# tzjtatata/Myriad

Hardware: AMD Instinct MI355X
Metric: images/sec fine-tune step (Vicuna-7B + LoRA-style adapters, 224px) (higher is better)
Workload: dtype bf16

## Files before the change

### include/myriad_hip.h

```cpp
#ifndef MYRIAD_HIP_H
#define MYRIAD_HIP_H
#include <stdint.h>

#ifdef __cplusplus
extern "C" {
#endif

typedef struct ihipStream_t* mh_stream_t;

#define MH_OK 0
#define MH_ERR_ARG (-1)
#define MH_ERR_LAUNCH (-2)
#define MH_ERR_UNSUPPORTED (-3)

#define MH_GEMM_OUT_F32 1
#define MH_GEMM_GELU 2
#define MH_GEMM_REGSTAGE 4

int mh_gemm_bf16_nt(const void* A, int lda, const void* B, int ldb, void* C, int ldc, int M, int N, int K,
                    const float* bias, const float* residual, int ldr, int flags, float alpha, mh_stream_t s);

int mh_gemm_plan(int M, int N, int K, int flags, int* kernel, int* splits);

int mh_prof_start(int capacity, mh_stream_t s);
// ... 111 lines not shown
int mh_lora_refresh_border(const float* Bq, const float* Bv, void* ext, long ld_ext, void* extT, long ld_extT, int W,
                           int D, int r, mh_stream_t st);
int mh_lora_refresh_borders(const void* table, int n_layers, long ld_ext, long ld_extT, int W, int D, int r, mh_stream_t stream);

int mh_lowrank_fwd(const float* x, const float* A, const float* Bm, float* y, float* t, int M, int D, int R,
                   mh_stream_t s);
long mh_lowrank_bwd_ws_floats(int M, int D, int R);
int mh_lowrank_bwd(const float* dy, const float* x, const float* t, const float* A, const float* Bm, float* dA,
                   float* dB, float* dx, float* ws, int M, int D, int R, mh_stream_t s);

int mh_clamp_ce(const float* logits, long ldl, const long* labels, float* row_loss, void* dlogits_bf16, long ldd,
                int R, int V, float grad_scale, mh_stream_t s);
int mh_sum_f32(const float* x, float* out, long n, float scale, mh_stream_t s);
int mh_argmax_rows(const float* logits, long ldl, long* out, float* margin, int R, int V, int ban_id, mh_stream_t s);
int mh_argmax_pmax_rows(const float* logits, long ldl, long* out, float* margin, float* pmax, int R, int V, int ban_id,
                        float inv_temp, mh_stream_t s);
int mh_decode_record(const long* nxt, const float* margin, const float* pmax, float* rec, long* next_ids, int* step, int R,
                     mh_stream_t s);
int mh_decode_advance(const long* nxt, const float* margin, const float* pmax, float* rec, long* next_ids, int* step, int* pos,
                      int* kvlen, int R, mh_stream_t s);
int mh_sample_rows(const float* logits, long ldl, long* out, float* margin, float* pmax, int* kept, float* u_out, int R, int V,
                   int ban_id, const float* params, const unsigned long long* seed, const int* step, int t_add, mh_stream_t s);
int mh_repetition_penalty_rows(float* logits, long ldl, unsigned* seen, const long* prev_ids, int R, int V, const float* penalty,
                               mh_stream_t s);
int mh_decode_advance_kept(const long* nxt, const float* margin, const float* pmax, const int* kept, float* rec, long* next_ids,
                           int* step, int* pos, int* kvlen, int R, mh_stream_t s);
int mh_decode_advance_rows(const long* nxt, const float* margin, const float* pmax, float* rec, long* next_ids, int* step,
                           int* pos, int* kvlen, const int* live, int R, mh_stream_t s);
int mh_sample_rows_slots(const float* logits, long ldl, long* out, float* margin, float* pmax, int* kept, float* u_out, int R, int V,
                         const float* params, const unsigned long long* seed, const int* gen, const int* live, mh_stream_t s);
int mh_argmax_pmax_rows_slots(const float* logits, long ldl, long* out, float* margin, float* pmax, int R, int V, const float* params,
                              const int* gen, const int* live, mh_stream_t s);
int mh_repetition_penalty_rows_slots(float* logits, long ldl, unsigned* seen, const long* prev_ids, int R, int V, const float* penalty,
                                     const int* live, mh_stream_t s);
int mh_decode_advance_kept_rows(const long* nxt, const float* margin, const float* pmax, const int* kept, float* rec, long* next_ids,
                                int* step, int* pos, int* kvlen, int* gen, const int* live, int R, mh_stream_t s);
int mh_token_scores_rows(const float* logits, long ldl, const long* ids, const int* watch, float* out, long ldo, int R, int V,
                         const int* live, mh_stream_t s);

int mh_beam_topk(const float* logits, long ldl, const float* scores, float* part_s, int* part_i, float* out_s, int* out_i, int B,
                 int rpi, int nb, int V, int ban_id, int* pos, int* kvlen, int n_adv, mh_stream_t s);
int mh_beam_reorder_kv(void* const* caches, int L, int B, int nb, long T_cap, int C, const int* src, const int* lo, const int* hi,
                       mh_stream_t s);

int mh_im2col_nhwc(const void* x, void* col, int B, int H, int W, int C, int kh, int kw, int pad, int Kpad,
                   mh_stream_t s);
int mh_col2im_nhwc(const void* dcol, float* dx, int B, int H, int W, int C, int kh, int kw, int pad, int Kpad,
                   mh_stream_t s);
int mh_relu_maxpool2_fwd(const void* y, int y_is_f32, long ldy, void* p, int B, int H, int W, int C, mh_stream_t s);
int mh_relu_maxpool2_bwd(const float* dp, const void* y, int y_is_f32, long ldy, void* dy, long lddy, int B, int H,
                         int W, int C, mh_stream_t s);
int mh_conv_pack_weight(const float* W, const float* bias, void* Wp, int Cout, int K, int Kpad, mh_stream_t s);
int mh_conv_unpack_grad(const float* dWp, float* dW, float* db, int Cout, int K, int Kpad, mh_stream_t s);

int mh_embed_gather(const void* table_bf16, const long* ids, const int* dst_rows, float* out, long n, int D, long ldo,
                    mh_stream_t s);
int mh_copy2d_f32(const float* src, long lds, float* dst, long ldd, long rows, int cols, int accumulate,
                  mh_stream_t s);
int mh_copy3d_f32(const float* src, long src_bstride, long lds, float* dst, long dst_bstride, long ldd, int nb,
                  long rows, int cols, int accumulate, mh_stream_t s);
int mh_gather_rows_f32_to_bf16(const float* src, long lds, const int* rows, void* dst, long n, int D, mh_stream_t s);
int mh_gather_rows_f32(const float* src, long lds, const int* rows, float* dst, long n, int D, mh_stream_t s);
int mh_gather_rows(const void* src, long lds, const int* rows, void* dst, long n, int D, int elem_bytes, mh_stream_t s);
int mh_expand_rows(const void* src, const int* inv, void* dst, long ldd, long M, int D, int elem_bytes, mh_stream_t s);
int mh_copy3d_bf16(const void* src, long src_bstride, long lds, void* dst, long dst_bstride, long ldd, int nb,
                   long rows, int cols, mh_stream_t s);
int mh_kv_append_bf16(const void* src, long ld_src, void* cache, long cache_bstride, long ld_cache, const int* pos_dev,
                      int B, int cols, mh_stream_t s);
int mh_rope_kv_append(void* qkv, long ld, int n_heads, int head_dim, const int* pos, const float* cos_tab,
                      const float* sin_tab, void* cache, long cache_bstride, long ld_cache, const int* pos_dev, int B,
                      mh_stream_t s);
int mh_add_i32(int* x, int n, int delta, mh_stream_t s);
long mh_gemv_pack_elems(int N, int K);
int mh_gemv_pack(const void* W, int ldb, int N, int K, void* out, mh_stream_t s);
int mh_gemv_packed(const void* A, int lda, const void* P, void* C, int ldc, int M, int N, int K, const float* bias,
                   const float* residual, int ldr, int out_f32, float alpha, mh_stream_t s);
int mh_gemv_packed_rmsnorm(const float* H, long ldh, const float* norm_w, float eps, const void* P, void* C, int ldc, int M,
                           int N, int K, const float* bias, const float* residual, int ldr, int out_f32, float alpha,
                           mh_stream_t s);
int mh_gemv_packed_silu(const void* gu, long ldgu, const void* P, void* C, int ldc, int M, int N, int K, const float* bias,
                        const float* residual, int ldr, int out_f32, float alpha, mh_stream_t s);
long mh_gemv_pack_fp8_elems(int N, int K);
int mh_gemv_pack_fp8(const void* W, int ldb, int N, int K, void* q_out, float* scale_out, mh_stream_t s);
int mh_gemv_packed_fp8(const void* A, int lda, const void* Q, const float* scale, void* C, int ldc, int M, int N, int K,
                       const float* bias, const float* residual, int ldr, int out_f32, float alpha, mh_stream_t s);
int mh_gemv_packed_fp8_rmsnorm(const float* H, long ldh, const float* norm_w, float eps, const void* Q, const float* scale,
                               void* C, int ldc, int M, int N, int K, const float* bias, const float* residual, int ldr,
                               int out_f32, float alpha, mh_stream_t s);
int mh_gemv_packed_fp8_silu(const void* gu, long ldgu, const void* Q, const float* scale, void* C, int ldc, int M, int N, int K,
                            const float* bias, const float* residual, int ldr, int out_f32, float alpha, mh_stream_t s);
long mh_gemv_pack_fp4_elems(int N, int K);
long mh_gemv_pack_fp4_scale_elems(int N, int K);
int mh_gemv_pack_fp4(const void* W, int ldb, int N, int K, void* q_out, void* scale_out, mh_stream_t s);
int mh_gemv_packed_fp4(const void* A, int lda, const void* Q, const void* scale, void* C, int ldc, int M, int N, int K,
                       const float* bias, const float* residual, int ldr, int out_f32, float alpha, mh_stream_t s);
int mh_gemv_packed_fp4_rmsnorm(const float* H, long ldh, const float* norm_w, float eps, const void* Q, const void* scale,
                               void* C, int ldc, int M, int N, int K, const float* bias, const float* residual, int ldr,
                               int out_f32, float alpha, mh_stream_t s);
int mh_gemv_packed_fp4_silu(const void* gu, long ldgu, const void* Q, const void* scale, void* C, int ldc, int M, int N, int K,
                            const float* bias, const float* residual, int ldr, int out_f32, float alpha, mh_stream_t s);
int mh_gemv_packed_wide(const void* A, int lda, const void* P, void* C, int ldc, int M, int N, int K, const float* bias,
                        const float* residual, int ldr, int out_f32, float alpha, mh_stream_t s);
int mh_gemv_packed_fp8_wide(const void* A, int lda, const void* Q, const float* scale, void* C, int ldc, int M, int N, int K,
                            const float* bias, const float* residual, int ldr, int out_f32, float alpha, mh_stream_t s);
int mh_gemv_packed_fp4_wide(const void* A, int lda, const void* Q, const void* scale, void* C, int ldc, int M, int N, int K,
                            const float* bias, const float* residual, int ldr, int out_f32, float alpha, mh_stream_t s);
// ... 112 lines not shown
```

### myriad_amd/build.py

```python
from __future__ import annotations

import os
import subprocess
import sys
from concurrent.futures import ThreadPoolExecutor

HERE = os.path.dirname(os.path.abspath(__file__))
CSRC = os.path.join(HERE, "csrc")
OBJ = os.path.join(CSRC, "build")
LIB = os.path.join(HERE, "libmyriad_hip.so")
LIB_DBG = os.path.join(HERE, "libmyriad_hip_dbg.so")
DBG_SOURCES = ["gemm", "gemm_256", "gemm_x4", "attn_seq", "lora"]
SOURCES = ["gemm", "gemm_256", "gemm_x4", "gemv", "attention", "attn_decode_split", "attn_ragged", "attn_seq", "attn_full", "norm", "elementwise", "conv", "loss", "sample", "scores", "beam", "lowrank", "lora", "expert", "image", "selfsup", "optim", "prof", "ctx", "wgrad", "qf_dropout", "lora_merge", "refresh", "version"]
FLAGS = ["--offload-arch=gfx950", "-O3", "-std=c++17", "-fPIC", "-ffp-contract=fast"]


def _stale(out, deps):
    if not os.path.exists(out):
        return True
    t = os.path.getmtime(out)
    return any(os.path.getmtime(d) > t for d in deps)


def build(force: bool = False, verbose: bool = True) -> str:
    hipcc = os.environ.get("HIPCC", "/opt/rocm/bin/hipcc")
    os.makedirs(OBJ, exist_ok=True)
    hdrs = [os.path.join(CSRC, h) for h in ("common.h", "gemv_pack.h", "attn_frag.h", "attn_tile.h")]
    gen, inc = os.path.join(CSRC, "gen_gemm_x4.py"), os.path.join(CSRC, "gemm_x4_loop.inc")
    if force or _stale(inc, [gen]):
        subprocess.check_call([sys.executable, gen])
    hdrs.append(inc)

    def one(job):
        name, dbg = job
        src = os.path.join(CSRC, name + ".hip")
        obj = os.path.join(OBJ, name + (".dbg.o" if dbg else ".o"))
        if force or _stale(obj, [src, *hdrs]):
            cmd = [hipcc, *FLAGS, *(["-DMH_DEBUG_HOOKS"] if dbg else []), "-c", src, "-o", obj]
            if verbose:
                print(" ".join(cmd), flush=True)
            subprocess.check_call(cmd)
        return obj

    jobs = [(n, False) for n in SOURCES] + [(n, True) for n in DBG_SOURCES]
    with ThreadPoolExecutor(max_workers=min(8, len(jobs))) as ex:
        built = dict(zip(jobs, ex.map(one, jobs)))
    objs = [built[(n, False)] for n in SOURCES]
    objs_dbg = [built[(n, n in DBG_SOURCES)] for n in SOURCES]
    for lib, oo in ((LIB, objs), (LIB_DBG, objs_dbg)):
        if force or _stale(lib, oo):
            cmd = [hipcc, "--offload-arch=gfx950", "-shared", "-fPIC", "-o", lib, *oo, "-ldl"]
            if verbose:
                print(" ".join(cmd), flush=True)
            subprocess.check_call(cmd)
    return LIB


if __name__ == "__main__":
    print(build(force="--force" in sys.argv))
```

### myriad_amd/csrc/common.h

```cpp
#pragma once
#include <hip/hip_runtime.h>
#include <stdint.h>

#define MH_OK 0
#define MH_ERR_ARG (-1)
#define MH_ERR_LAUNCH (-2)
#define MH_ERR_UNSUPPORTED (-3)

typedef unsigned short bf16_t;
typedef __attribute__((ext_vector_type(8))) short short8_t;
typedef __attribute__((ext_vector_type(4))) short short4_t;
typedef __attribute__((ext_vector_type(4))) float float4_t;
typedef __attribute__((ext_vector_type(16))) float float16_t;

#define MH_CHECK_LAUNCH()                                   \
  do {                                                      \
    hipError_t e__ = hipGetLastError();                     \
    if (e__ != hipSuccess) return MH_ERR_LAUNCH;            \
  } while (0)

#define MH_MAX_ALT_WS 4
struct MhScratch {
  float* ws;
  size_t bytes;
  float* alt[MH_MAX_ALT_WS];
  hipStream_t alt_stream[MH_MAX_ALT_WS];
};
extern MhScratch g_default_scratch;
extern MhScratch* g_scratch;

enum MhOpt {
  MH_OPT_SLAB_BF16 = 0,
  MH_OPT_GEMM_SKINNY,
  MH_OPT_SWIGLU_FUSED,
  MH_OPT_GELU_FUSED,
  MH_OPT_ATTN_BWD_SPLIT,
  MH_OPT_GEMM_ZERO_PAD,
  MH_OPT_GEMM256_IMPL,
  MH_OPT_LORA_NORM_FUSED,
  MH_OPT_ATTN_FULL,
  MH_OPT_LORA_WGRAD_MFMA,
  MH_OPT_GEMM_SKIP_PAD,
  MH_OPT_GEMM_SPLIT_XCD,
  MH_OPT_COUNT
};
int mh_opt(int id);

extern bool g_mh_prof_on;
void mh_prof_pre(hipStream_t s, int kernel, int M, int N, int K, int splits, int flags);
void mh_prof_post(hipStream_t s);

__device__ __forceinline__ float bf2f(bf16_t h) { return __uint_as_float(((unsigned)h) << 16); }

typedef __bf16 mh_bf2_t __attribute__((ext_vector_type(2)));
typedef float mh_f2_t __attribute__((ext_vector_type(2)));
__device__ __forceinline__ bf16_t f2bf_sw(float f) {
  unsigned u = __float_as_uint(f);
  if ((u & 0x7fffffffu) > 0x7f800000u) return (bf16_t)((u >> 16) | 0x40);
  u += 0x7fffu + ((u >> 16) & 1u);
  return (bf16_t)(u >> 16);
}
__device__ __forceinline__ bf16_t f2bf(float f) {
  const __bf16 b = (__bf16)f;
  return (bf16_t)__builtin_bit_cast(unsigned short, b);
}
__device__ __forceinline__ unsigned pack_bf2(float lo, float hi) {
  const mh_f2_t v = {lo, hi};
  const mh_bf2_t b = __builtin_convertvector(v, mh_bf2_t);
  return __builtin_bit_cast(unsigned, b);
}

__device__ __forceinline__ unsigned dropout_hash(unsigned long long seed, unsigned long long idx) {
  unsigned h = (unsigned)idx * 0x9E3779B1u + ((unsigned)seed ^ ((unsigned)(idx >> 32) * 0x85EBCA77u));
  h ^= (unsigned)(seed >> 32) & 0x7FFFFFFFu;
  h ^= h >> 16;
  h *= 0x85EBCA6Bu;
  h ^= h >> 13;
  h *= 0xC2B2AE35u;
  h ^= h >> 16;
  return h;
}
__device__ __forceinline__ unsigned dropout_hash2(unsigned h) {
  h = (h ^ 0x68E31DA4u) * 0x2C1B3C6Du;
  return h ^ (h >> 15);
}
__device__ __forceinline__ float dropout_keep(unsigned long long seed, unsigned long long idx, float p, float inv_keep) {
  if (p <= 0.f) return 1.f;
  unsigned h = dropout_hash(seed, idx);
  if (seed >> 63) h = dropout_hash2(h);
  const float u = (float)(h >> 8) * (1.0f / 16777216.0f);
  return u >= p ? inv_keep : 0.f;
}
__device__ __forceinline__ void dropout_keep_pair(unsigned long long seed, unsigned long long idx, float p, float inv_keep,
                                                  float& k0, float& k1) {
  if (p <= 0.f) { k0 = k1 = 1.f; return; }
  const unsigned h = dropout_hash(seed, idx);
// ... 85 lines not shown
```

### myriad_amd/csrc/version.hip

```cpp
#include "common.h"
#include <stdlib.h>
#include <string.h>
extern "C" const char* mh_version(void) { return "myriad_hip 0.1 (gfx950)"; }
extern "C" int mh_target_arch(void) { return 950; }

struct MhOptEntry { const char* name; const char* env; int def; int value; };
static MhOptEntry g_opts[MH_OPT_COUNT] = {
    {"slab_bf16", "MYRIAD_SLAB_BF16", 1, -1},
    {"gemm_skinny", "MYRIAD_GEMM_SKINNY", 1, -1},
    {"swiglu_fused", "MYRIAD_SWIGLU_FUSED", 1, -1},
    {"gelu_fused", "MYRIAD_GELU_FUSED", 1, -1},
    {"attn_bwd_split", "MYRIAD_ATTN_BWD_SPLIT", 1, -1},
    {"gemm_zero_pad", "MYRIAD_GEMM_ZERO_PAD", 1, -1},
    {"gemm256_impl", "MYRIAD_GEMM256_IMPL", 1, -1},
    {"lora_norm_fused", "MYRIAD_LORA_NORM_FUSED", 1, -1},
    {"attn_full", "MYRIAD_ATTN_FULL", 1, -1},
    {"lora_wgrad_mfma", "MYRIAD_LORA_WGRAD_MFMA", 1, -1},
    {"gemm_skip_pad", "MYRIAD_GEMM_SKIP_PAD", 1, -1},
    {"gemm_split_xcd", "MYRIAD_GEMM_SPLIT_XCD", 1, -1},
};

int mh_opt(int id) {
  MhOptEntry& o = g_opts[id];
  if (o.value < 0) {
    const char* e = getenv(o.env);
    o.value = e ? (e[0] == '0' ? 0 : 1) : o.def;
  }
  return o.value;
}

static int find_opt(const char* name) {
  if (!name) return -1;
  for (int i = 0; i < MH_OPT_COUNT; ++i)
    if (!strcmp(name, g_opts[i].name)) return i;
  return -1;
}
extern "C" int mh_get_option(const char* name) {
  const int i = find_opt(name);
  return i < 0 ? MH_ERR_ARG : mh_opt(i);
}
extern "C" int mh_set_option(const char* name, int value) {
  const int i = find_opt(name);
  if (i < 0 || (value != 0 && value != 1)) return MH_ERR_ARG;
  const int prev = mh_opt(i);
  g_opts[i].value = value;
  return prev;
}
```

### myriad_amd/networks.py

```python
from __future__ import annotations

from typing import Dict, List, Optional, Tuple

import torch

from . import ops

BF16, F32 = torch.bfloat16, torch.float32

STEM_CH = [(1, 4), (4, 16), (16, 64), (64, 256), (256, 1024)]
STEM_IDX = (0, 3, 6, 9, 12)


def ve_param_specs(prefix: str, head_out: int, head_k: int) -> List[Tuple[str, Tuple[int, ...], Tuple[int, ...]]]:
    specs = []
    for idx, (ci, co) in zip(STEM_IDX, STEM_CH):
        specs.append((f"{prefix}meta_net.{idx}.weight", (co, 9 * ci), (co, ci, 3, 3)))
        specs.append((f"{prefix}meta_net.{idx}.bias", (co,), (co,)))
    specs.append((f"{prefix}meta_net.15.weight", (head_out, head_k * head_k * 1024), (head_out, 1024, head_k, head_k)))
    specs.append((f"{prefix}meta_net.15.bias", (head_out,), (head_out,)))
    return specs


def from_reference_layout(t: torch.Tensor, internal_shape) -> torch.Tensor:
    if t.dim() == 4 and len(internal_shape) != 4:
        return t.permute(0, 2, 3, 1).reshape(internal_shape).contiguous()
    return t.reshape(internal_shape).contiguous()


def to_reference_layout(t: torch.Tensor, ref_shape) -> torch.Tensor:
    if len(ref_shape) == 4 and t.dim() != 4:
        co, ci, kh, kw = ref_shape
        return t.reshape(co, kh, kw, ci).permute(0, 3, 1, 2).contiguous()
    return t.reshape(ref_shape).contiguous()


class VENet:

    def __init__(self, prefix: str, head_k: int, head_out: int, params: Dict[str, torch.Tensor],
                 grads: Dict[str, torch.Tensor], device):
        self.prefix, self.head_k, self.head_out = prefix, head_k, head_out
        self.p, self.g, self.dev = params, grads, torch.device(device)
        self._saved = None

    def _w(self, idx):
        return self.p[f"{self.prefix}meta_net.{idx}.weight"], self.p[f"{self.prefix}meta_net.{idx}.bias"]

    def forward(self, maps: torch.Tensor, save_for_backward: bool = True) -> torch.Tensor:
        B, _, H, W = maps.shape
        x = ops.to_bf16(maps.contiguous()).view(B, H, W, 1)
        saved = []
        for idx, (ci, co) in zip(STEM_IDX, STEM_CH):
            wm, bias = self._w(idx)
            wp = ops.conv_pack(wm, bias)
            col = ops.im2col(x, 3, 3, 1)
            y = ops.gemm(col, wp, out_dtype=F32)
            saved.append((col, y, wp, H, W, ci, co))
            x = ops.relu_pool_fwd(y, B, H, W, co)
            H, W = H // 2, W // 2
        wm, bias = self._w(15)
        if self.head_k == 1:
            x2 = x.view(B * H * W, 1024)
            wb = ops.to_bf16(wm)
            out = ops.gemm(x2, wb, bias=bias, out_dtype=F32)
            head = (x2, wb, None, True)
            T = H * W
        else:
            k = self.head_k
            T = (H - k + 1) * (W - k + 1)
            if wm.shape[1] % 64 == 0:
                wp = ops.to_bf16(wm)
                col = ops.im2col(x, k, k, 0, bias_col=False)
                out = ops.gemm(col, wp, bias=bias, out_dtype=F32)
                head = (col, wp, (H, W), True)
            else:
                wp = ops.conv_pack(wm, bias)
                col = ops.im2col(x, k, k, 0)
                out = ops.gemm(col, wp, out_dtype=F32)
                head = (col, wp, (H, W), False)
        if save_for_backward:
            self._saved = dict(stem=saved, head=head, B=B)
        return out.view(B, T, self.head_out)

    @property
    def head_accumulates_in_place(self) -> bool:
        return self.head_k != 1 and (self.head_k * self.head_k * 1024) % 64 == 0

    def backward(self, dtokens: torch.Tensor, accumulate_head: bool = False) -> None:
        sv = self._saved
        if sv is None:
            raise RuntimeError("backward() without saved forward")
        B = sv["B"]
        dy32 = dtokens.reshape(-1, self.head_out).contiguous()
        dyb = ops.to_bf16(dy32)
        gw, gb = self.g[f"{self.prefix}meta_net.15.weight"], self.g[f"{self.prefix}meta_net.15.bias"]
        a, wq, hw = sv["head"][:3]
        dyT = ops.transpose_to_bf16(dyb, 64)
        if self.head_k == 1:
            ops.gemm_auto_f32(dyT, ops.transpose_to_bf16(a, 64), gw)
            gb.copy_(ops.colsum(dy32))
            dp = ops.gemm(dyb, ops.transpose_to_bf16(wq, 64), out_dtype=F32)
        else:
            Kpad = wq.shape[1]
            if sv["head"][3]:
                if accumulate_head:
                    ops.gemm(dyT, ops.transpose_to_bf16(a, 64), out=gw, residual=gw)
                else:
                    ops.gemm_auto_f32(dyT, ops.transpose_to_bf16(a, 64), gw)
                gb.copy_(ops.colsum(dy32))
            else:
                dwp = torch.empty((self.head_out, Kpad), dtype=F32, device=self.dev)
                ops.gemm_auto_f32(dyT, ops.transpose_to_bf16(a, 64), dwp)
                ops.conv_unpack_grad(dwp, gw, gb)
            dcol = ops.gemm(dyb, ops.transpose_to_bf16(wq, 64))
            H, W = hw
            dp = ops.col2im(dcol, B, H, W, 1024, self.head_k, self.head_k, 0)
        for li in range(4, -1, -1):
            col, y, wp, H, W, ci, co = sv["stem"][li]
            idx = STEM_IDX[li]
            dy, dyfull = ops.relu_pool_bwd(dp, y, B, H, W, co, pad_cols_to=64)
            dwp = torch.empty((co, wp.shape[1]), dtype=F32, device=self.dev)
            ops.gemm_auto_f32(ops.transpose_to_bf16(dy, 64), ops.transpose_to_bf16(col, 64), dwp)
            ops.conv_unpack_grad(dwp, self.g[f"{self.prefix}meta_net.{idx}.weight"],
                                 self.g[f"{self.prefix}meta_net.{idx}.bias"])
            if li > 0:
                wpT = ops.transpose_to_bf16(wp, 64)
                dcol = ops.gemm(dyfull, wpT)
                dp = ops.col2im(dcol, B, H, W, ci, 3, 3, 1)
        self._saved = None


class LoraAdaptor:

    def __init__(self, params, grads, prefix="expert_adaptor."):
        self.A, self.Bm = params[prefix + "conv1.weight"], params[prefix + "conv2.weight"]
        self.gA, self.gB = grads[prefix + "conv1.weight"], grads[prefix + "conv2.weight"]
        self._saved = None

    def forward(self, x2d: torch.Tensor, save_for_backward=True):
        y, t = ops.lowrank_fwd(x2d, self.A, self.Bm)
        if save_for_backward:
            self._saved = (x2d, t)
        return y

    def backward(self, dy2d: torch.Tensor, need_dx: bool = False):
        x2d, t = self._saved
        dx = ops.lowrank_bwd(dy2d, x2d, t, self.A, self.Bm, self.gA, self.gB, need_dx=need_dx)
        self._saved = None
        return dx
```

### myriad_amd/ops.py

```python
from __future__ import annotations

import math
import numbers
from typing import Optional

import os

import torch

from . import _lib

BF16 = torch.bfloat16
F32 = torch.float32

GEMM_OUT_F32 = 1
GEMM_GELU = 2
GEMM_REGSTAGE = 4
GEMM_VARIANT = 0


def _L():
    return _lib.load()


# ... 1209 lines not shown
    _chk_flat(lo, torch.int32, 1, "beam_reorder_kv: lo")
    _chk_flat(hi, torch.int32, 1, "beam_reorder_kv: hi")
    _lib.check(_L().mh_beam_reorder_kv(_p(cache_table), L, B, nb, int(T_cap), C, _p(src), _p(lo), _p(hi), _s()),
               "mh_beam_reorder_kv")


def im2col(x_nhwc: torch.Tensor, kh: int, kw: int, pad: int, bias_col: bool = True):
    B, H, W, C = x_nhwc.shape
    OH, OW = H + 2 * pad - kh + 1, W + 2 * pad - kw + 1
    Kpad = round_up(kh * kw * C + (1 if bias_col else 0), 64)
    if not bias_col and Kpad != kh * kw * C:
        raise _lib.MyriadHipError(f"im2col: bias_col=False needs kh*kw*C % 64 == 0, got {kh * kw * C}")
    col = torch.empty((B * OH * OW, Kpad), dtype=BF16, device=x_nhwc.device)
    _lib.check(_L().mh_im2col_nhwc(_p(x_nhwc), _p(col), B, H, W, C, kh, kw, pad, Kpad, _s()), "mh_im2col_nhwc")
    return col


def col2im(dcol: torch.Tensor, B, H, W, C, kh, kw, pad):
    dx = torch.empty((B, H, W, C), dtype=F32, device=dcol.device)
    _lib.check(_L().mh_col2im_nhwc(_p(dcol), _p(dx), B, H, W, C, kh, kw, pad, dcol.stride(0), _s()), "mh_col2im_nhwc")
    return dx


def relu_pool_fwd(y2d: torch.Tensor, B, H, W, C):
    p = torch.empty((B, H // 2, W // 2, C), dtype=BF16, device=y2d.device)
    _lib.check(_L().mh_relu_maxpool2_fwd(_p(y2d), int(y2d.dtype == F32), y2d.stride(0), _p(p), B, H, W, C, _s()),
               "mh_relu_maxpool2_fwd")
    return p


def relu_pool_bwd(dp: torch.Tensor, y2d: torch.Tensor, B, H, W, C, pad_cols_to: int = 1):
    cpad = round_up(C, pad_cols_to)
    full = (torch.zeros if cpad != C else torch.empty)((B * H * W, cpad), dtype=BF16, device=y2d.device)
    _lib.check(_L().mh_relu_maxpool2_bwd(_p(dp), _p(y2d), int(y2d.dtype == F32), y2d.stride(0), _p(full),
                                         full.stride(0), B, H, W, C, _s()), "mh_relu_maxpool2_bwd")
    return full[:, :C], full


def conv_pack(Wm: torch.Tensor, bias: Optional[torch.Tensor], out=None):
    Cout, K = Wm.shape
    Kpad = round_up(K + 1, 64)
    if out is None:
        out = torch.empty((Cout, Kpad), dtype=BF16, device=Wm.device)
    _lib.check(_L().mh_conv_pack_weight(_p(Wm), _p(bias), _p(out), Cout, K, Kpad, _s()), "mh_conv_pack_weight")
    return out


def conv_unpack_grad(dWp: torch.Tensor, dW: torch.Tensor, db: Optional[torch.Tensor]):
    Cout, Kpad = dWp.shape
    K = dW.shape[1]
    _lib.check(_L().mh_conv_unpack_grad(_p(dWp), _p(dW), _p(db), Cout, K, Kpad, _s()), "mh_conv_unpack_grad")


def adamw_step(p, g, m, v, lr, wd, step, beta1=0.9, beta2=0.999, eps=1e-8, grad_scale=1.0, shadow=None):
    _lib.check(_L().mh_adamw_step(_p(p), _p(g), _p(m), _p(v), _p(shadow), p.numel(), float(lr), float(beta1),
                                  float(beta2), float(eps), float(wd), int(step), float(grad_scale), _s()),
               "mh_adamw_step")


def adamw_gated(p, g, m, v, lr, wd, used: torch.Tensor, steps: torch.Tensor, beta1=0.9, beta2=0.999, eps=1e-8, grad_scale=1.0):
    _lib.check(_L().mh_adamw_gated(_p(p), _p(g), _p(m), _p(v), p.numel(), float(lr), float(beta1), float(beta2), float(eps),
                                   float(wd), float(grad_scale), _p(used), _p(steps), _s()), "mh_adamw_gated")


def adamw_bump(used: torch.Tensor, steps: torch.Tensor):
    _lib.check(_L().mh_adamw_bump(_p(used), _p(steps), steps.numel(), _s()), "mh_adamw_bump")


def grad_sumsq_slots(n: int) -> int:
    return int(_L().mh_grad_sumsq_slots(int(n)))


def grad_sumsq(g: torch.Tensor, used: torch.Tensor, partials: torch.Tensor) -> int:
    _lib.check(_L().mh_grad_sumsq(_p(g), g.numel(), _p(used), _p(partials), partials.numel(), _s()), "mh_grad_sumsq")
    return grad_sumsq_slots(g.numel())


def clip_rank_sum(partials: torch.Tensor, n_partials: int, rank_sums: torch.Tensor, rank: int):
    _lib.check(_L().mh_clip_rank_sum(_p(partials), int(n_partials), _p(rank_sums), rank_sums.numel(), int(rank), _s()),
               "mh_clip_rank_sum")


def clip_finalize(partials: torch.Tensor, n_partials: int, rank_sums: Optional[torch.Tensor], max_norm: Optional[float],
                  grad_scale: float, guard: bool, ctl: torch.Tensor):
    if n_partials > partials.numel() or ctl.numel() < 4 or ctl.dtype != torch.float64 or partials.dtype != torch.float64:
        raise _lib.MyriadHipError("clip_finalize: f64 partials / ctl[4] expected")
    _lib.check(_L().mh_clip_finalize(_p(partials), int(n_partials), _p(rank_sums), 0 if rank_sums is None else rank_sums.numel(),
                                     float("inf") if max_norm is None else float(max_norm), float(grad_scale), int(bool(guard)),
                                     _p(ctl), _s()), "mh_clip_finalize")


def adamw_gated_ctl(p, g, m, v, lr, wd, used: torch.Tensor, steps: torch.Tensor, ctl: torch.Tensor, beta1=0.9, beta2=0.999, eps=1e-8):
    _lib.check(_L().mh_adamw_gated_ctl(_p(p), _p(g), _p(m), _p(v), p.numel(), float(lr), float(beta1), float(beta2), float(eps),
                                       float(wd), _p(used), _p(steps), _p(ctl), _s()), "mh_adamw_gated_ctl")


def adamw_bump_ctl(used: torch.Tensor, steps: torch.Tensor, ctl: torch.Tensor):
    _lib.check(_L().mh_adamw_bump_ctl(_p(used), _p(steps), steps.numel(), _p(ctl), _s()), "mh_adamw_bump_ctl")


def l2norm_rows(x: torch.Tensor, want_bf16: bool = True, want_f32: bool = False, eps: float = 1e-12):
    _chk2d(x, F32, "l2norm_rows.x")
    M, D = x.shape
    yb = torch.empty((M, D), dtype=BF16, device=x.device) if want_bf16 else None
    yf = torch.empty((M, D), dtype=F32, device=x.device) if want_f32 else None
    _lib.check(_L().mh_l2norm_rows(_p(x), x.stride(0), _p(yb), _p(yf), D, M, D, float(eps), _s()), "mh_l2norm_rows")
# ... 59 lines not shown
```

Measured before the change: 206.5.

## Fuse stem conv3x3 with ReLU and maxpool in forward and backward

Adds dedicated HIP kernels for the small-channel stem convolutions (1→4, 4→16, 16→64). The forward kernel builds im2col patches on the fly in registers, runs MFMA, and writes both the pre-activation and the pooled output. The backward pass fuses pool/ReLU gradient recovery into a split-K wgrad kernel, followed by a reduction kernel and a tiled dx kernel. This replaces the im2col, packing, transposes and separate GEMM launches with fewer kernels and less memory traffic. The path is gated by a runtime option that defaults on.

Result: no change. 207.0, median of 5 (+0.2%).

```diff
diff --git a/include/myriad_hip.h b/include/myriad_hip.h
--- a/include/myriad_hip.h
+++ b/include/myriad_hip.h
@@ -187,6 +187,12 @@
                          int W, int C, mh_stream_t s);
 int mh_conv_pack_weight(const float* W, const float* bias, void* Wp, int Cout, int K, int Kpad, mh_stream_t s);
 int mh_conv_unpack_grad(const float* dWp, float* dW, float* db, int Cout, int K, int Kpad, mh_stream_t s);
+
+int mh_conv3x3_relu_pool_fwd(const void* x, const float* W, const float* bias, float* y, void* p, int B, int H, int Wd, int ci,
+                             int co, mh_stream_t s);
+long mh_conv3x3_relu_pool_bwd_ws_floats(int B, int H, int Wd, int ci, int co);
+int mh_conv3x3_relu_pool_bwd(const float* dp, const float* y, const void* x, const float* W, float* dW, float* db, float* dx,
+                             float* ws, long ws_floats, int B, int H, int Wd, int ci, int co, mh_stream_t s);
 
 int mh_embed_gather(const void* table_bf16, const long* ids, const int* dst_rows, float* out, long n, int D, long ldo,
                     mh_stream_t s);
diff --git a/myriad_amd/build.py b/myriad_amd/build.py
--- a/myriad_amd/build.py
+++ b/myriad_amd/build.py
@@ -11,7 +11,7 @@
 LIB = os.path.join(HERE, "libmyriad_hip.so")
 LIB_DBG = os.path.join(HERE, "libmyriad_hip_dbg.so")
 DBG_SOURCES = ["gemm", "gemm_256", "gemm_x4", "attn_seq", "lora"]
-SOURCES = ["gemm", "gemm_256", "gemm_x4", "gemv", "attention", "attn_decode_split", "attn_ragged", "attn_seq", "attn_full", "norm", "elementwise", "conv", "loss", "sample", "scores", "beam", "lowrank", "lora", "expert", "image", "selfsup", "optim", "prof", "ctx", "wgrad", "qf_dropout", "lora_merge", "refresh", "version"]
+SOURCES = ["gemm", "gemm_256", "gemm_x4", "gemv", "attention", "attn_decode_split", "attn_ragged", "attn_seq", "attn_full", "norm", "elementwise", "conv", "conv_stem", "loss", "sample", "scores", "beam", "lowrank", "lora", "expert", "image", "selfsup", "optim", "prof", "ctx", "wgrad", "qf_dropout", "lora_merge", "refresh", "version"]
 FLAGS = ["--offload-arch=gfx950", "-O3", "-std=c++17", "-fPIC", "-ffp-contract=fast"]
 
 
diff --git a/myriad_amd/csrc/common.h b/myriad_amd/csrc/common.h
--- a/myriad_amd/csrc/common.h
+++ b/myriad_amd/csrc/common.h
@@ -42,6 +42,7 @@
   MH_OPT_LORA_WGRAD_MFMA,
   MH_OPT_GEMM_SKIP_PAD,
   MH_OPT_GEMM_SPLIT_XCD,
+  MH_OPT_CONV_STEM,
   MH_OPT_COUNT
 };
 int mh_opt(int id);
diff --git a/myriad_amd/csrc/conv_stem.hip b/myriad_amd/csrc/conv_stem.hip
--- /dev/null
+++ b/myriad_amd/csrc/conv_stem.hip
@@ -0,0 +1,458 @@
+#include "common.h"
+#include "gemv_pack.h"
+
+extern "C" int mh_gemm_plan(int M, int N, int K, int flags, int* kernel, int* splits);
+
+struct StemWalk { int gv; int per; int chains; };
+
+static bool stem_walk(int M, int N, int K, int flags, StemWalk* w) {
+  int kernel = 1, splits = 1;
+  if (mh_gemm_plan(M, N, K, flags, &kernel, &splits) != MH_OK) return false;
+  const int nsteps = K / 64;
+  if (kernel == 0) {
+    const int nw = gv_packed_nw(N);
+    w->gv = 1;
+    w->per = (nsteps + nw - 1) / nw;
+    w->chains = (nsteps + w->per - 1) / w->per;
+    return true;
+  }
+  if (splits != 1) return false;
+  *w = {0, nsteps, 1};
+  return true;
+}
+
+__device__ __forceinline__ int stem_k0(int gv, int t, int lg) {
+  return gv ? (t >> 1) * 64 + lg * 16 + (t & 1) * 8 : t * 32 + lg * 8;
+}
+__device__ __forceinline__ float4_t stem_mfma(int gv, short8_t wside, short8_t aside, float4_t acc) {
+  return gv ? __builtin_amdgcn_mfma_f32_16x16x32_bf16(aside, wside, acc, 0, 0, 0)
+            : __builtin_amdgcn_mfma_f32_16x16x32_bf16(wside, aside, acc, 0, 0, 0);
+}
+
+#define ST_LD 72
+
+__device__ __forceinline__ bf16_t stem_wp(const float* __restrict__ Wm, const float* __restrict__ bias, int co, int K, int n,
+                                          int k) {
+  if (n >= co || k > K) return 0;
+  return f2bf(k < K ? Wm[(long)n * K + k] : bias[n]);
+}
+
+template <int CI>
+__device__ __forceinline__ short8_t stem_patch(const bf16_t* __restrict__ xb, int H, int W, int oy, int ox, int k0, bool live) {
+  constexpr int K = 9 * CI;
+  short8_t v = {0, 0, 0, 0, 0, 0, 0, 0};
+  if (!live) return v;
+  if constexpr (CI % 8 == 0) {
+    if (k0 + 8 <= K) {
+      const int tap = k0 / CI, c = k0 - tap * CI, ky = tap / 3, kx = tap - ky * 3;
+      const int iy = oy + ky - 1, ix = ox + kx - 1;
+      if (iy >= 0 && iy < H && ix >= 0 && ix < W) v = *reinterpret_cast<const short8_t*>(xb + ((long)iy * W + ix) * CI + c);
+      return v;
+    }
+  }
+#pragma unroll
+  for (int j = 0; j < 8; ++j) {
+    const int k = k0 + j;
+    short e = 0;
+    if (k < K) {
+      const int tap = k / CI, c = k - tap * CI, ky = tap / 3, kx = tap - ky * 3;
+      const int iy = oy + ky - 1, ix = ox + kx - 1;
+      if (iy >= 0 && iy < H && ix >= 0 && ix < W) e = (short)xb[((long)iy * W + ix) * CI + c];
+    } else if (k == K) {
+      e = 0x3F80;
+    }
+    v[j] = e;
+  }
+  return v;
+}
+
+template <int CO>
+__device__ __forceinline__ void stem_dy4(const float* __restrict__ dp, const float* __restrict__ y, int H, int W, int b, int oy,
+                                         int ox, int n0, bf16_t (&out)[4]) {
+  const long base = ((long)b * H + (oy & ~1)) * W + (ox & ~1);
+  const float4_t v0 = *reinterpret_cast<const float4_t*>(y + base * CO + n0);
+  const float4_t v1 = *reinterpret_cast<const float4_t*>(y + (base + 1) * CO + n0);
+  const float4_t v2 = *reinterpret_cast<const float4_t*>(y + (base + W) * CO + n0);
+  const float4_t v3 = *reinterpret_cast<const float4_t*>(y + (base + W + 1) * CO + n0);
+  const float4_t g = *reinterpret_cast<const float4_t*>(dp + (((long)b * (H >> 1) + (oy >> 1)) * (W >> 1) + (ox >> 1)) * CO + n0);
+  const int self = (oy & 1) * 2 + (ox & 1);
+#pragma unroll
+  for (int c = 0; c < 4; ++c) {
+    float best = v0[c];
+    int arg = 0;
+    if (v1[c] > best) { best = v1[c]; arg = 1; }
+    if (v2[c] > best) { best = v2[c]; arg = 2; }
+    if (v3[c] > best) { best = v3[c]; arg = 3; }
+    out[c] = (arg == self && best > 0.f) ? f2bf(g[c]) : (bf16_t)0;
+  }
+}
+
+template <int CI, int CO, int FPW>
+__global__ __launch_bounds__(256) void conv_stem_fwd_kernel(const bf16_t* __restrict__ x, const float* __restrict__ Wm,
+                                                            const float* __restrict__ bias, float* __restrict__ y,
+                                                            bf16_t* __restrict__ p, int B, int H, int W, int gv, int per) {
+  constexpr int K = 9 * CI, KP = (K + 1 + 63) / 64 * 64, NT32 = KP / 32, NB = (CO + 15) / 16, CH = NB * 16;
+  __shared__ __attribute__((aligned(16))) bf16_t wl[CH][KP + 8];
+  __shared__ float tile[4][FPW][16][CH + 1];
+  const int tid = threadIdx.x, lane = tid & 63, wave = tid >> 6, lr = lane & 15, lg = lane >> 4;
+  if constexpr (K % 4 != 0) {
+    for (int i = tid; i < CH * KP; i += 256) {
+      const int n = i / KP, k = i - n * KP;
+      wl[n][k] = stem_wp(Wm, bias, CO, K, n, k);
+    }
+  } else {
+    static_assert(K % 4 != 0 || CH == CO, "whole fragments of channels");
+    for (int i = tid; i < CO * (K / 4); i += 256) {
+      const int n = i / (K / 4), k = (i - n * (K / 4)) * 4;
+      const float4_t w4 = *reinterpret_cast<const float4_t*>(Wm + (long)n * K + k);
+      uint2 pk;
+      pk.x = pack_bf2(w4[0], w4[1]);
+      pk.y = pack_bf2(w4[2], w4[3]);
+      *reinterpret_cast<uint2*>(&wl[n][k]) = pk;
+    }
+    for (int i = tid; i < CH * (KP - K); i += 256) {
+      const int n = i / (KP - K), k = K + (i - n * (KP - K));
+      wl[n][k] = stem_wp(Wm, bias, CO, K, n, k);
+    }
+  }
+  __syncthreads();
+  const int PH = H >> 1, PW = W >> 1, cw = (W + 7) >> 3;
+  const long frags = (long)B * PH * cw;
+  const long per_it = (long)gridDim.x * 4 * FPW;
+  const long iters = (frags + per_it - 1) / per_it;
+  const int cl = gv ? 2 * per : NT32;
+  for (long it = 0; it < iters; ++it) {
+    const long f0 = ((it * gridDim.x + blockIdx.x) * 4 + wave) * FPW;
+    short8_t xf[FPW][NT32];
+#pragma unroll
+    for (int fp = 0; fp < FPW; ++fp) {
+      const long f = f0 + fp;
+      const bool live_f = f < frags;
+      const int c8 = (int)(f % cw), py = (int)((f / cw) % PH), b = (int)(f / ((long)cw * PH));
+      const int oy = 2 * py + (lr >> 3), ox = c8 * 8 + (lr & 7);
+      const bf16_t* xb = x + (long)(live_f ? b : 0) * H * W * CI;
+#pragma unroll
+      for (int t = 0; t < NT32; ++t)
+        if (gv || t * 32 <= K) xf[fp][t] = stem_patch<CI>(xb, H, W, oy, ox, stem_k0(gv, t, lg), live_f && ox < W);
+    }
+#pragma unroll
+    for (int fp = 0; fp < FPW; ++fp) {
+      float4_t acc[NB], tot[NB];
+#pragma unroll
+      for (int nb = 0; nb < NB; ++nb) acc[nb] = tot[nb] = (float4_t){0.f, 0.f, 0.f, 0.f};
+#pragma unroll
+      for (int t = 0; t < NT32; ++t) {
+        if (gv || t * 32 <= K) {
+          const int k0 = stem_k0(gv, t, lg);
+#pragma unroll
+          for (int nb = 0; nb < NB; ++nb)
+            acc[nb] = stem_mfma(gv, *reinterpret_cast<const short8_t*>(&wl[nb * 16 + lr][k0]), xf[fp][t], acc[nb]);
+        }
+        if ((t + 1) % cl == 0 || t == NT32 - 1) {
+#pragma unroll
+          for (int nb = 0; nb < NB; ++nb) {
+#pragma unroll
+            for (int e = 0; e < 4; ++e) tot[nb][e] += acc[nb][e];
+            acc[nb] = (float4_t){0.f, 0.f, 0.f, 0.f};
+          }
+        }
+      }
+#pragma unroll
+      for (int nb = 0; nb < NB; ++nb)
+#pragma unroll
+        for (int e = 0; e < 4; ++e) {
+          if (gv) tile[wave][fp][lg * 4 + e][nb * 16 + lr] = tot[nb][e];
+          else tile[wave][fp][lr][nb * 16 + lg * 4 + e] = tot[nb][e];
+        }
+    }
+    __syncthreads();
+#pragma unroll
+    for (int fp = 0; fp < FPW; ++fp) {
+      const long f = f0 + fp;
+      if (f >= frags) break;
+      const int c8 = (int)(f % cw), py = (int)((f / cw) % PH), b = (int)(f / ((long)cw * PH));
+#pragma unroll
+      for (int ii = 0; ii < 16 * CO / 64; ++ii) {
+        const int i = lane + ii * 64;
+        const int px = i / CO, ch = i - px * CO;
+        const int yy = 2 * py + (px >> 3), xx = c8 * 8 + (px & 7);
+        if (xx < W) y[(((long)b * H + yy) * W + xx) * CO + ch] = tile[wave][fp][px][ch];
+      }
+#pragma unroll
+      for (int ii = 0; ii < (4 * CO + 63) / 64; ++ii) {
+        const int i = lane + ii * 64;
+        const int q = i / CO, ch = i - q * CO, pxo = c8 * 4 + q;
+        if (i < 4 * CO && pxo < PW) {
+          float m = 0.f;
+          m = fmaxf(m, tile[wave][fp][2 * q][ch]);
+          m = fmaxf(m, tile[wave][fp][2 * q + 1][ch]);
+          m = fmaxf(m, tile[wave][fp][8 + 2 * q][ch]);
+          m = fmaxf(m, tile[wave][fp][8 + 2 * q + 1][ch]);
+          p[(((long)b * PH + py) * PW + pxo) * CO + ch] = f2bf(m);
+        }
+      }
+    }
+    __syncthreads();
+  }
+}
+
+template <int CI, int CO, int RT>
+__global__ __launch_bounds__(256) void conv_stem_wgrad_kernel(const float* __restrict__ dp, const float* __restrict__ y,
+                                                              const bf16_t* __restrict__ x, float* __restrict__ ws, int B, int H,
+                                                              int W, int gv, int tps, int kt) {
+  constexpr int K = 9 * CI, KB = (K + 1 + 15) / 16, FR = (KB + 3) / 4, RP = RT * 64, LD = RP + 8, PARTS = 256 / RP;
+  constexpr int NQ = (CO < 16 ? CO : 16) / 4;
+  constexpr int NU = CI == 1 ? 9 : (CI == 4 ? 9 : 18);
+  __shared__ __attribute__((aligned(16))) bf16_t colL[KB * 16][LD];
+  __shared__ __attribute__((aligned(16))) bf16_t dyL[16][LD];
+  const int tid = threadIdx.x, lane = tid & 63, wave = tid >> 6, lr = lane & 15, lg = lane >> 4;
+  const long M = (long)B * H * W;
+  const int chain = blockIdx.x, nb = blockIdx.y;
+  const int t0 = chain * tps, t1 = (t0 + tps) < kt ? (t0 + tps) : kt;
+  for (int i = tid; i < (KB * 16 - K - 1) * LD; i += 256) colL[K + 1 + i / LD][i % LD] = 0;
+  for (int i = tid; i < (16 - NQ * 4) * LD; i += 256) dyL[NQ * 4 + i / LD][i % LD] = 0;
+  const int r = tid % RP, part = tid / RP;
+  float4_t acc[FR];
+#pragma unroll
+  for (int i = 0; i < FR; ++i) acc[i] = (float4_t){0.f, 0.f, 0.f, 0.f};
+  for (int tl = t0; tl < t1; tl += RT) {
+    const int nt = (t1 - tl) < RT ? (t1 - tl) : RT;
+    const long m = (long)tl * 64 + r;
+    const bool live = r < nt * 64 && m < M;
+    const int ox = live ? (int)(m % W) : 0, oy = live ? (int)((m / W) % H) : 0, b = live ? (int)(m / ((long)W * H)) : 0;
+    __syncthreads();
+#pragma unroll
+    for (int uu = 0; uu < (NU + PARTS - 1) / PARTS; ++uu) {
+      const int u = part + uu * PARTS;
+      if (u >= NU) break;
+      const int tap = CI == 16 ? (u >> 1) : u, c0 = CI == 16 ? (u & 1) * 8 : 0, ky = tap / 3, kx = tap - ky * 3;
+      const int iy = oy + ky - 1, ix = ox + kx - 1;
+      const bool in = live && iy >= 0 && iy < H && ix >= 0 && ix < W;
+      const bf16_t* src = x + (((long)b * H + iy) * W + ix) * CI + c0;
+      if constexpr (CI == 1) {
+        colL[tap][r] = in ? *src : (bf16_t)0;
+      } else if constexpr (CI == 4) {
+        uint2 v = {0u, 0u};
+        if (in) v = *reinterpret_cast<const uint2*>(src);
+        colL[tap * 4 + 0][r] = (bf16_t)(v.x & 0xffffu); colL[tap * 4 + 1][r] = (bf16_t)(v.x >> 16);
+        colL[tap * 4 + 2][r] = (bf16_t)(v.y & 0xffffu); colL[tap * 4 + 3][r] = (bf16_t)(v.y >> 16);
+      } else {
+        short8_t v = {0, 0, 0, 0, 0, 0, 0, 0};
+        if (in) v = *reinterpret_cast<const short8_t*>(src);
+#pragma unroll
+        for (int j = 0; j < 8; ++j) colL[tap * 16 + c0 + j][r] = (bf16_t)v[j];
+      }
+    }
+    if (part == 0) colL[K][r] = live ? (bf16_t)0x3F80 : (bf16_t)0;
+#pragma unroll
+    for (int qq = 0; qq < (NQ + PARTS - 1) / PARTS; ++qq) {
+      const int q = part + qq * PARTS;
+      if (q >= NQ) break;
+      bf16_t d[4] = {0, 0, 0, 0};
+      if (live) stem_dy4<CO>(dp, y, H, W, b, oy, ox, nb * 16 + q * 4, d);
+#pragma unroll
+      for (int c = 0; c < 4; ++c) dyL[q * 4 + c][r] = d[c];
+    }
+    __syncthreads();
+    for (int tt = 0; tt < nt; ++tt) {
+#pragma unroll
+      for (int s = 0; s < 2; ++s) {
+        const int k0 = tt * 64 + (gv ? lg * 16 + s * 8 : s * 32 + lg * 8);
+        const short8_t df = *reinterpret_cast<const short8_t*>(&dyL[lr][k0]);
+#pragma unroll
+        for (int i = 0; i < FR; ++i) {
+          const int kb = wave + 4 * i;
+          if (kb < KB) acc[i] = stem_mfma(gv, *reinterpret_cast<const short8_t*>(&colL[kb * 16 + lr][k0]), df, acc[i]);
+        }
+      }
+    }
+  }
+  float* out = ws + (long)chain * CO * (K + 1);
+#pragma unroll
+  for (int i = 0; i < FR; ++i) {
+    const int kb = wave + 4 * i;
+    if (kb < KB) {
+#pragma unroll
+      for (int e = 0; e < 4; ++e) {
+        const int n = nb * 16 + (gv ? lg * 4 + e : lr), kc = kb * 16 + (gv ? lr : lg * 4 + e);
+        if (n < CO && kc <= K) out[(long)n * (K + 1) + kc] = acc[i][e];
+      }
+    }
+  }
+}
+
+__global__ __launch_bounds__(256) void conv_stem_wsum_kernel(const float* __restrict__ ws, float* __restrict__ dW,
+                                                             float* __restrict__ db, int co, int K, int chains) {
+  const int lane = threadIdx.x & 63;
+  const int total = co * (K + 1);
+  const int o = blockIdx.x * 4 + (threadIdx.x >> 6);
+  if (o >= total) return;
+  float s = 0.f;
+  for (int c0 = 0; c0 < chains; c0 += 512) {
+    int v[8];
+#pragma unroll
+    for (int u = 0; u < 8; ++u) {
+      const int c = c0 + u * 64 + lane;
+      v[u] = __float_as_int(c < chains ? ws[(long)c * total + o] : 0.f);
+    }
+#pragma unroll
+    for (int u = 0; u < 8; ++u) {
+      if (c0 + u * 64 >= chains) break;
+#pragma unroll
+      for (int j = 0; j < 64; ++j) s += __int_as_float(__builtin_amdgcn_readlane(v[u], j));
+    }
+  }
+  if (lane == 0) {
+    const int n = o / (K + 1), kc = o - n * (K + 1);
+    if (kc < K) dW[(long)n * K + kc] = s;
+    else db[n] = s;
+  }
+}
+
+template <int CI, int CO>
+__global__ __launch_bounds__(256) void conv_stem_dx_kernel(const float* __restrict__ dp, const float* __restrict__ y,
+                                                           const float* __restrict__ Wm, float* __restrict__ dx, int B, int H, int W,
+                                                           int gv) {
+  constexpr int K = 9 * CI, QN = CO / 4;
+  __shared__ __attribute__((aligned(16))) bf16_t dyL[100][ST_LD];
+  __shared__ __attribute__((aligned(16))) bf16_t wT[K][ST_LD];
+  const int tid = threadIdx.x, lane = tid & 63, wave = tid >> 6, lr = lane & 15, lg = lane >> 4;
+  const int tw = (W + 7) >> 3, th = (H + 7) >> 3;
+  const int tx = blockIdx.x % tw, ty = (blockIdx.x / tw) % th, b = blockIdx.x / (tw * th);
+  const int y0 = ty * 8, x0 = tx * 8;
+  if constexpr (CO < 64) {
+    for (int i = tid; i < (100 + K) * (64 - CO); i += 256) {
+      const int row = i / (64 - CO), n = CO + i % (64 - CO);
+      if (row < 100) dyL[row][n] = 0;
+      else wT[row - 100][n] = 0;
+    }
+  }
+  for (int i = tid; i < CO * (K / 4); i += 256) {
+    const int n = i / (K / 4), k = (i - n * (K / 4)) * 4;
+    const float4_t w4 = *reinterpret_cast<const float4_t*>(Wm + (long)n * K + k);
+#pragma unroll
+    for (int j = 0; j < 4; ++j) wT[k + j][n] = f2bf(w4[j]);
+  }
+  for (int i = tid; i < 100 * QN; i += 256) {
+    const int hp = i / QN, q = i - hp * QN;
+    const int oy = y0 - 1 + hp / 10, ox = x0 - 1 + hp % 10;
+    bf16_t d[4] = {0, 0, 0, 0};
+    if (oy >= 0 && oy < H && ox >= 0 && ox < W) stem_dy4<CO>(dp, y, H, W, b, oy, ox, q * 4, d);
+    uint2 pk;
+    pk.x = (unsigned)d[0] | ((unsigned)d[1] << 16);
+    pk.y = (unsigned)d[2] | ((unsigned)d[3] << 16);
+    *reinterpret_cast<uint2*>(&dyL[hp][q * 4]) = pk;
+  }
+  __syncthreads();
+  const int ly = wave * 2 + (lr >> 3), lx = lr & 7;
+  float s[4] = {0.f, 0.f, 0.f, 0.f};
+#pragma unroll
+  for (int ky = 0; ky < 3; ++ky)
+#pragma unroll
+    for (int kx = 0; kx < 3; ++kx) {
+      const int hp = (ly + 2 - ky) * 10 + (lx + 2 - kx);
+      const int wrow = (ky * 3 + kx) * CI + (lr & (CI - 1));
+      float4_t acc = (float4_t){0.f, 0.f, 0.f, 0.f};
+#pragma unroll
+      for (int t = 0; t < 2; ++t) {
+        if (gv || t * 32 < CO) {
+          const int k0 = stem_k0(gv, t, lg);
+          acc = stem_mfma(gv, *reinterpret_cast<const short8_t*>(&wT[wrow][k0]),
+                          *reinterpret_cast<const short8_t*>(&dyL[hp][k0]), acc);
+        }
+      }
+#pragma unroll
+      for (int e = 0; e < 4; ++e) s[e] += bf2f(f2bf(acc[e]));
+    }
+  if (gv) {
+    if (lr < CI) {
+#pragma unroll
+      for (int e = 0; e < 4; ++e) {
+        const int px = lg * 4 + e, iy = y0 + wave * 2 + (px >> 3), ix = x0 + (px & 7);
+        if (iy < H && ix < W) dx[(((long)b * H + iy) * W + ix) * CI + lr] = s[e];
+      }
+    }
+  } else {
+    const int iy = y0 + ly, ix = x0 + lx;
+    if (lg * 4 < CI && iy < H && ix < W)
+      *reinterpret_cast<float4_t*>(dx + (((long)b * H + iy) * W + ix) * CI + lg * 4) = (float4_t){s[0], s[1], s[2], s[3]};
+  }
+}
+
+static bool stem_shape_ok(int B, int H, int W, int ci, int co) {
+  return B > 0 && H > 0 && W > 0 && !(H & 1) && !(W & 1) && (long)B * H * W < (1L << 31);
+}
+static bool stem_layer_ok(int ci, int co) { return (ci == 1 && co == 4) || (ci == 4 && co == 16) || (ci == 16 && co == 64); }
+
+extern "C" int mh_conv3x3_relu_pool_fwd(const void* x, const float* W, const float* bias, float* y, void* p, int B, int H,
+                                        int Wd, int ci, int co, hipStream_t stream) {
+  if (!x || !W || !bias || !y || !p || !stem_shape_ok(B, H, Wd, ci, co)) return MH_ERR_ARG;
+  if (!stem_layer_ok(ci, co)) return MH_ERR_UNSUPPORTED;
+  const int Kpad = (9 * ci + 1 + 63) / 64 * 64;
+  StemWalk w;
+  if (!stem_walk(B * H * Wd, co, Kpad, 1, &w)) return MH_ERR_UNSUPPORTED;
+  const long frags = (long)B * (H / 2) * ((Wd + 7) / 8);
+  const int fpw = ci == 16 ? 1 : 4;
+  long g = (frags + 4 * fpw - 1) / (4 * fpw);
+  if (g > 2048) g = 2048;
+#define ST_FWD(CI_, CO_)                                                                                                   \
+  hipLaunchKernelGGL((conv_stem_fwd_kernel<CI_, CO_, CI_ == 16 ? 1 : 4>), dim3((int)g), dim3(256), 0, stream, (const bf16_t*)x, W, bias, y,    \
+                     (bf16_t*)p, B, H, Wd, w.gv, w.per)
+  if (ci == 1) ST_FWD(1, 4);
+  else if (ci == 4) ST_FWD(4, 16);
+  else ST_FWD(16, 64);
+#undef ST_FWD
+  MH_CHECK_LAUNCH();
+  return MH_OK;
+}
+
+static bool stem_wgrad_walk(int M, int ci, int co, StemWalk* w) {
+  const int Kpad = (9 * ci + 1 + 63) / 64 * 64;
+  const int kt = (M + 63) / 64;
+  const int tiles = ((co + 127) / 128) * ((Kpad + 127) / 128);
+  if (tiles >= 128 || kt < 16) return stem_walk(co, Kpad, kt * 64, 1, w);
+  int splits = kt / 4 < 512 / tiles ? kt / 4 : 512 / tiles;
+  if (splits < 1) splits = 1;
+  if (splits > kt) splits = kt;
+  const int tps = (kt + splits - 1) / splits;
+  *w = {0, tps, (kt + tps - 1) / tps};
+  return true;
+}
+
+extern "C" long mh_conv3x3_relu_pool_bwd_ws_floats(int B, int H, int Wd, int ci, int co) {
+  StemWalk w;
+  if (!stem_shape_ok(B, H, Wd, ci, co) || !stem_layer_ok(ci, co) || !stem_wgrad_walk(B * H * Wd, ci, co, &w)) return 0;
+  return (long)w.chains * co * (9 * ci + 1);
+}
+
+extern "C" int mh_conv3x3_relu_pool_bwd(const float* dp, const float* y, const void* x, const float* W, float* dW, float* db,
+                                        float* dx, float* ws, long ws_floats, int B, int H, int Wd, int ci, int co,
+                                        hipStream_t stream) {
+  if (!dp || !y || !x || !W || !dW || !db || !ws || !stem_shape_ok(B, H, Wd, ci, co)) return MH_ERR_ARG;
+  if (!stem_layer_ok(ci, co)) return MH_ERR_UNSUPPORTED;
+  if (dx && ((uintptr_t)dx & 15)) return MH_ERR_ARG;
+  const int M = B * H * Wd, K = 9 * ci, Kpad = (K + 1 + 63) / 64 * 64;
+  StemWalk ww, wd = {0, 1, 1};
+  if (!stem_wgrad_walk(M, ci, co, &ww)) return MH_ERR_UNSUPPORTED;
+  if (dx && (ci == 1 || !stem_walk(M, Kpad, 64, 0, &wd))) return MH_ERR_UNSUPPORTED;
+  if (ws_floats < (long)ww.chains * co * (K + 1)) return MH_ERR_ARG;
+  const int kt = (M + 63) / 64;
+#define ST_WG(CI_, CO_, RT_)                                                                                               \
+  hipLaunchKernelGGL((conv_stem_wgrad_kernel<CI_, CO_, RT_>), dim3(ww.chains, (CO_ + 15) / 16), dim3(256), 0, stream, dp, y,  \
+                     (const bf16_t*)x, ws, B, H, Wd, ww.gv, ww.per, kt)
+  if (ci == 1) ST_WG(1, 4, 4);
+  else if (ci == 4) ST_WG(4, 16, 4);
+  else ST_WG(16, 64, 1);
+#undef ST_WG
+  MH_CHECK_LAUNCH();
+  hipLaunchKernelGGL(conv_stem_wsum_kernel, dim3((co * (K + 1) + 3) / 4), dim3(256), 0, stream, (const float*)ws, dW, db, co, K,
+                     ww.chains);
+  MH_CHECK_LAUNCH();
+  if (dx) {
+    const dim3 grid(B * ((H + 7) / 8) * ((Wd + 7) / 8));
+    if (ci == 4) hipLaunchKernelGGL((conv_stem_dx_kernel<4, 16>), grid, dim3(256), 0, stream, dp, y, W, dx, B, H, Wd, wd.gv);
+    else hipLaunchKernelGGL((conv_stem_dx_kernel<16, 64>), grid, dim3(256), 0, stream, dp, y, W, dx, B, H, Wd, wd.gv);
+    MH_CHECK_LAUNCH();
+  }
+  return MH_OK;
+}
diff --git a/myriad_amd/csrc/version.hip b/myriad_amd/csrc/version.hip
--- a/myriad_amd/csrc/version.hip
+++ b/myriad_amd/csrc/version.hip
@@ -18,6 +18,7 @@
     {"lora_wgrad_mfma", "MYRIAD_LORA_WGRAD_MFMA", 1, -1},
     {"gemm_skip_pad", "MYRIAD_GEMM_SKIP_PAD", 1, -1},
     {"gemm_split_xcd", "MYRIAD_GEMM_SPLIT_XCD", 1, -1},
+    {"conv_stem", "MYRIAD_CONV_STEM", 1, -1},
 };
 
 int mh_opt(int id) {
diff --git a/myriad_amd/networks.py b/myriad_amd/networks.py
--- a/myriad_amd/networks.py
+++ b/myriad_amd/networks.py
@@ -50,8 +50,15 @@
         B, _, H, W = maps.shape
         x = ops.to_bf16(maps.contiguous()).view(B, H, W, 1)
         saved = []
+        fused = ops.conv_stem_enabled()
         for idx, (ci, co) in zip(STEM_IDX, STEM_CH):
             wm, bias = self._w(idx)
+            if fused and ops.conv_stem_eligible(ci, co):
+                y, p = ops.conv3x3_relu_pool_fwd(x, wm, bias)
+                saved.append((None, y, x, H, W, ci, co))
+                x = p
+                H, W = H // 2, W // 2
+                continue
             wp = ops.conv_pack(wm, bias)
             col = ops.im2col(x, 3, 3, 1)
             y = ops.gemm(col, wp, out_dtype=F32)
@@ -118,6 +125,11 @@
         for li in range(4, -1, -1):
             col, y, wp, H, W, ci, co = sv["stem"][li]
             idx = STEM_IDX[li]
+            if col is None:
+                dp = ops.conv3x3_relu_pool_bwd(dp.contiguous(), y, wp, self.p[f"{self.prefix}meta_net.{idx}.weight"],
+                                               self.g[f"{self.prefix}meta_net.{idx}.weight"],
+                                               self.g[f"{self.prefix}meta_net.{idx}.bias"], need_dx=li > 0)
+                continue
             dy, dyfull = ops.relu_pool_bwd(dp, y, B, H, W, co, pad_cols_to=64)
             dwp = torch.empty((co, wp.shape[1]), dtype=F32, device=self.dev)
             ops.gemm_auto_f32(ops.transpose_to_bf16(dy, 64), ops.transpose_to_bf16(col, 64), dwp)
diff --git a/myriad_amd/ops.py b/myriad_amd/ops.py
--- a/myriad_amd/ops.py
+++ b/myriad_amd/ops.py
@@ -1285,6 +1285,60 @@
     _lib.check(_L().mh_conv_unpack_grad(_p(dWp), _p(dW), _p(db), Cout, K, Kpad, _s()), "mh_conv_unpack_grad")
 
 
+def conv_stem_enabled() -> bool:
+    return _L().mh_get_option(b"conv_stem") == 1
+
+
+def set_conv_stem(on: bool) -> bool:
+    return _L().mh_set_option(b"conv_stem", int(bool(on))) == 1
+
+
+def conv_stem_eligible(ci: int, co: int) -> bool:
+    return (ci, co) in ((1, 4), (4, 16), (16, 64))
+
+
+def conv3x3_relu_pool_fwd(x_nhwc: torch.Tensor, Wm: torch.Tensor, bias: torch.Tensor, y=None, p=None):
+    B, H, W, ci = x_nhwc.shape
+    co = Wm.shape[0]
+    if x_nhwc.dtype != BF16 or not x_nhwc.is_contiguous() or Wm.dtype != F32 or tuple(Wm.shape) != (co, 9 * ci) or not Wm.is_contiguous() \
+            or bias.dtype != F32 or bias.numel() != co:
+        raise _lib.MyriadHipError(f"conv3x3_relu_pool_fwd: need x bf16 NHWC contiguous, W f32 [co, 9 ci], bias f32 [co]; got "
+                                  f"{x_nhwc.dtype} {tuple(x_nhwc.shape)}, {Wm.dtype} {tuple(Wm.shape)}, {bias.dtype} {tuple(bias.shape)}")
+    if (H | W) & 1:
+        raise _lib.MyriadHipError(f"conv3x3_relu_pool_fwd: H and W must be even, got {H} x {W}")
+    if y is None:
+        y = torch.empty((B * H * W, co), dtype=F32, device=x_nhwc.device)
+    if p is None:
+        p = torch.empty((B, H // 2, W // 2, co), dtype=BF16, device=x_nhwc.device)
+    _lib.check(_L().mh_conv3x3_relu_pool_fwd(_p(x_nhwc), _p(Wm), _p(bias), _p(y), _p(p), B, H, W, ci, co, _s()),
+               f"mh_conv3x3_relu_pool_fwd B={B} H={H} W={W} ci={ci} co={co}")
+    return y, p
+
+
+def conv3x3_relu_pool_bwd(dp: torch.Tensor, y: torch.Tensor, x_nhwc: torch.Tensor, Wm: torch.Tensor, dW: torch.Tensor,
+                          db: torch.Tensor, need_dx: bool = True, dx=None):
+    B, H, W, ci = x_nhwc.shape
+    co = Wm.shape[0]
+    if dp.dtype != F32 or not dp.is_contiguous() or dp.numel() != B * (H // 2) * (W // 2) * co or y.dtype != F32 or not y.is_contiguous() \
+            or y.numel() != B * H * W * co or x_nhwc.dtype != BF16 or not x_nhwc.is_contiguous():
+        raise _lib.MyriadHipError("conv3x3_relu_pool_bwd: need contiguous dp f32 [B,H/2,W/2,co], y f32 [B*H*W, co], x bf16 [B,H,W,ci]")
+    if dW.dtype != F32 or not dW.is_contiguous() or tuple(dW.shape) != (co, 9 * ci) or db.dtype != F32 or not db.is_contiguous() \
+            or db.numel() != co:
+        raise _lib.MyriadHipError("conv3x3_relu_pool_bwd: dW must be contiguous f32 [co, 9 ci], db contiguous f32 [co]")
+    if (H | W) & 1:
+        raise _lib.MyriadHipError(f"conv3x3_relu_pool_bwd: H and W must be even, got {H} x {W}")
+    nws = int(_L().mh_conv3x3_relu_pool_bwd_ws_floats(B, H, W, ci, co))
+    if nws <= 0:
+        raise _lib.MyriadHipError(f"conv3x3_relu_pool_bwd: unsupported layer B={B} H={H} W={W} ci={ci} co={co}")
+    ws = torch.empty((nws,), dtype=F32, device=y.device)
+    if need_dx and dx is None:
+        dx = torch.empty((B, H, W, ci), dtype=F32, device=y.device)
+    _lib.check(_L().mh_conv3x3_relu_pool_bwd(_p(dp), _p(y), _p(x_nhwc), _p(Wm), _p(dW), _p(db), _p(dx) if need_dx else None, _p(ws),
+                                             nws, B, H, W, ci, co, _s()),
+               f"mh_conv3x3_relu_pool_bwd B={B} H={H} W={W} ci={ci} co={co}")
+    return dx if need_dx else None
+
+
 def adamw_step(p, g, m, v, lr, wd, step, beta1=0.9, beta2=0.999, eps=1e-8, grad_scale=1.0, shadow=None):
     _lib.check(_L().mh_adamw_step(_p(p), _p(g), _p(m), _p(v), _p(shadow), p.numel(), float(lr), float(beta1),
                                   float(beta2), float(eps), float(wd), int(step), float(grad_scale), _s()),
```
